# inhavl-shlee/AFI-GAN

Measured on AMD Instinct MI355X. Metric: stage1_G+D_step_images_per_s, higher is better.
Workload: dtype f32 via f16x3: two scaled fp16 pieces per operand, three f16 MFMAs per product, fp32 accumulate (tensors fp32)

## Files before the change

afigan_amd/csrc/afi_launch.h:

```cpp
#pragma once
#include "afi_common.h"

int afi_launch_pix_gemm(const AfiPixGemm& p, int b_rc, hipStream_t st);
int afi_launch_gemm_tn(const float* Q, const float* V, float* dU, int planes, long long rows_per_plane, int M, int N, hipStream_t st, bool deterministic = false);
int afi_launch_gemm_nt(const float* A, const float* B, float* C, int planes, long long rows_per_plane, int N, int K, hipStream_t st);
int afi_launch_split_bf16_tiles(const float* B, void* out, int planes, int N, int K, int split, hipStream_t st);
int afi_launch_gemm_nt_bf16_dma(const float* A, const void* Bsplit, float* C, int planes, long long rows_per_plane, int N, int K, int split, hipStream_t st);
int afi_launch_gemm_tn_bf16(const float* Q, const float* V, float* dU, int planes, long long rows_per_plane, int M, int N, int split, hipStream_t st, bool deterministic = false);
int afi_launch_split_f16_tiles(const float* B, void* out, int planes, int N, int K, hipStream_t st, int wkind = 0);
int afi_f16_image_begin(void* out, hipStream_t st);
float* afi_f16_image_wmax(void* out);
long long afi_f16_image_bytes(int planes, int N, int K);
int afi_launch_absmax_planes(const float* X, long long per_plane, int planes, float* out, hipStream_t st);
AfiF16Bound afi_f16_bound(const float* amax, int kind);
int afi_launch_gemm_nt_f16x3(const float* A, const void* Bimg, float* C, int planes, long long rows_per_plane, int N, int K, const AfiF16Bound& ab, hipStream_t st,
                             bool a_pre = false, long long nt256_min_tiles = 512, bool local_sums = false);
int afi_launch_gemm_tn_f16x3(const float* Q, const float* V, float* dU, int planes, long long rows_per_plane, int M, int N, const AfiF16Bound& qb, const AfiF16Bound& vb,
                             hipStream_t st, bool pre = false, bool deterministic = false);
int afi_launch_wgrad_gemm(const AfiWgradGemm& p, hipStream_t st);
int afi_launch_wgrad_gemm_group(const AfiWgradGemm* probs, int n, int wide, hipStream_t st);
int afi_launch_wgrad_gemm_group6(const AfiWgradGemm* probs, int n, hipStream_t st);
int afi_launch_pix_gemm_group(const AfiPixGemm* probs, int n, int b_rc, hipStream_t st);
void* afi_prof_open(hipStream_t st, int kind, double flops, long long m, int n, int k);
void afi_prof_close(void* scope);

long long afi_wk6_image_bytes(int Ncols, int Ck, int ntaps, int nKphase);
int afi_launch_wk6_images(const AfiWk6ImgJob* jobs, int n, hipStream_t st, const AfiWk6Side* side = nullptr, const AfiWk6ConvT* ct = nullptr);
int afi_launch_pix_gemm_sk(const AfiPixGemm& p, int b_rc, hipStream_t st);
int afi_launch_pix_gemm_wk_group(const AfiPixGemm* probs, int n, int b_rc, hipStream_t st);
int afi_launch_wgrad_group(const AfiWgradGemm* probs, int n, int wide, hipStream_t st);
int afi_launch_wgrad6_group(const AfiWgradGemm* probs, int n, hipStream_t st);

#define AFI_FROZEN1X1_PLAN_SLOTS 12
enum { AFI_F1_M = 0, AFI_F1_BM, AFI_F1_BN, AFI_F1_KC, AFI_F1_NTM, AFI_F1_NTN, AFI_F1_GRID, AFI_F1_LDS, AFI_F1_XBYTES, AFI_F1_OBYTES, AFI_F1_IBYTES, AFI_F1_XDENSE };

int afi_launch_nchw_to_nhwc(const float* in, float* out, int N, int C, int P, hipStream_t st);
int afi_launch_cast_to_f32_nhwc(const void* in, int dt, int N, int C, int H, int W, long long sN, long long sC, long long sH, long long sW, float* out,
                                hipStream_t st);
int afi_launch_cast_from_f32_nhwc(const AfiView& in, int N, int H, int W, int C, void* out, int dt, hipStream_t st);

int afi_launch_colsum_group(const AfiColsumProb* probs, int n, hipStream_t st);
int afi_launch_nhwc_to_nchw(const float* in, float* out, int N, int C, int P, hipStream_t st);
int afi_launch_convT_pack(const float* W, float* Wp, int Cin, int Cout, hipStream_t st);
int afi_launch_convT_unpack_grad(const float* dWp, float* dW, int Cin, int Cout, hipStream_t st);
int afi_launch_rdb_wgrad_unpack(const float* dWp, float* const dw[4], int C, int G, float alpha, hipStream_t st);
int afi_launch_rdb_wgrad_unpack_multi(const float* dWp, long long stride, float* const (*dw)[4], int nblocks, int C, int G, float alpha, hipStream_t st);
int afi_launch_g_bwd_tail(const AfiColsumProb* cs, int n_cs, const float* dWpT, float* dWT, int Cin, int Cout,
                          const float* dWp, long long stride, float* const (*dw)[4], int nblocks, int C, int G, float alpha, hipStream_t st);
int afi_launch_rdb_xpart_pack(const float* const w[4], float* out, int C, int G, hipStream_t st);
// ... 58 lines not shown
```

afigan_amd/csrc/frozen1x1.hip:

```cpp
#include "afi_common.h"
#include "afi_launch.h"
#include "afi_bf16_split.h"

#define AFI_F1_ROWS 64
struct AfiFrozen1x1 {
    const float* x; long long x_sN, x_sH, x_sW;
    const unsigned char* image; const float* bias; const float* add; float* out;
    unsigned x_bytes, o_bytes, i_bytes;
    int x_dense, M, HW, W, Cin, Cout, kc, ntile_n, nst;
    float alpha, add_scale; int act;
};

__device__ __forceinline__ int afi_f1_logical_id() {
    const int nwg = gridDim.x, qq = nwg >> 3, rr = nwg & 7, xcd = blockIdx.x & 7;
    return (xcd < rr ? xcd * (qq + 1) : rr * (qq + 1) + (xcd - rr) * qq) + (int)(blockIdx.x >> 3);
}

template <int NJ>
__global__ __launch_bounds__(256, 2) void afi_frozen1x1_kernel(const AfiFrozen1x1 p) {
    extern __shared__ __attribute__((aligned(16))) unsigned char lds[];
    const int tid = threadIdx.x, lane = tid & 63, l15 = lane & 15, lq = lane >> 4;
    const int wave = __builtin_amdgcn_readfirstlane(tid >> 6);
    const int lb = afi_f1_logical_id();
    const int tile_m = lb / p.ntile_n, tile_n = lb - tile_m * p.ntile_n;
    const int m0 = tile_m * AFI_F1_ROWS;
    const int kc = p.kc, nks = kc >> 5, nchunks = p.Cin / kc, part_bytes = kc * 128;
    const int pl = kc == 128 ? 5 : (kc == 64 ? 4 : 3);
    const int iters = 1 << (pl - 2);
    const __amdgpu_buffer_rsrc_t rsrc_x = __builtin_amdgcn_make_buffer_rsrc((void*)p.x, 0, p.x_bytes, 0x00020000);
    const __amdgpu_buffer_rsrc_t rsrc_b = __builtin_amdgcn_make_buffer_rsrc((void*)p.image, 0, p.i_bytes, 0x00020000);

    const int q = tid & ((1 << pl) - 1), r0 = tid >> pl, rstep = 256 >> pl;
    unsigned row_off[8];
// ... 79 lines not shown
                for (int mi = 0; mi < 4; ++mi) acc[j][mi] = mfma(bm, fa[mi][1], acc[j][mi]);
#pragma unroll
                for (int mi = 0; mi < 4; ++mi) acc[j][mi] = mfma(bh, fa[mi][1], acc[j][mi]);
#pragma unroll
                for (int mi = 0; mi < 4; ++mi) acc[j][mi] = mfma(bm, fa[mi][0], acc[j][mi]);
#pragma unroll
                for (int mi = 0; mi < 4; ++mi) acc[j][mi] = mfma(bh, fa[mi][0], acc[j][mi]);
            }
        }
        if (c + 1 < nchunks) __syncthreads();
    }

    const __amdgpu_buffer_rsrc_t rsrc_o = __builtin_amdgcn_make_buffer_rsrc((void*)p.out, 0, p.o_bytes, 0x00020000);
    const __amdgpu_buffer_rsrc_t rsrc_r = __builtin_amdgcn_make_buffer_rsrc((void*)p.add, 0, p.add ? p.o_bytes : 0u, 0x00020000);
    const float slope = p.act == 1 ? AFI_LRELU_SLOPE : 0.f;
#pragma unroll
    for (int j = 0; j < NJ; ++j) {
        const int col = 16 * (h0 + j) + 4 * lq;
        if (16 * (h0 + j) >= p.Cout) break;
        f32x4 bias = {0.f, 0.f, 0.f, 0.f};
        if (p.bias) bias = *(const f32x4*)(p.bias + col);
        unsigned off[4];
        f32x4 r[4];
#pragma unroll
        for (int mi = 0; mi < 4; ++mi) {
            const int m = m0 + 16 * mi + l15;
            off[mi] = m < p.M ? 4u * ((unsigned)m * (unsigned)p.Cout + (unsigned)col) : 0xFFFFFFFFu;
            r[mi] = f32x4{0.f, 0.f, 0.f, 0.f};
            if (p.add) r[mi] = __builtin_bit_cast(f32x4, __builtin_amdgcn_raw_buffer_load_b128(rsrc_r, off[mi], 0, 0));
        }
#pragma unroll
        for (int mi = 0; mi < 4; ++mi) {
            f32x4 v = p.alpha * acc[j][mi];
            v += bias;
            if (p.add) v += p.add_scale * r[mi];
            if (p.act) {
#pragma unroll
                for (int e = 0; e < 4; ++e) v[e] = v[e] > 0.f ? v[e] : v[e] * slope;
            }
            __builtin_amdgcn_raw_buffer_store_b128(__builtin_bit_cast(u32x4, v), rsrc_o, off[mi], 0, 0);
        }
    }
}

extern "C" int afi_frozen1x1_plan(int N, int H, int W, int Cin, int Cout, long long x_sN, long long x_sH, long long x_sW, long long o_sN, long long o_sH,
                                  long long o_sW, int has_add, long long a_sN, long long a_sH, long long a_sW, long long* plan) {
    if (!plan || N <= 0 || H <= 0 || W <= 0 || Cin <= 0 || Cout <= 0) return AFI_ERR_BAD_ARG;
    for (int i = 0; i < AFI_FROZEN1X1_PLAN_SLOTS; ++i) plan[i] = 0;
    if ((Cin & 31) || (Cout & 31)) return AFI_ERR_UNSUPPORTED;
    const long long kLimit = 0x7FFFFFF0LL;
    const long long M = (long long)N * H * W;
    if (M > (1LL << 30)) return AFI_ERR_UNSUPPORTED;
    if (x_sW < Cin || x_sW % Cin != 0) return AFI_ERR_UNSUPPORTED;
    const long long s = x_sW / Cin, row_span = ((long long)(W - 1) * s + 1) * Cin;
    if (H > 1 && x_sH < s * row_span) return AFI_ERR_UNSUPPORTED;
// ... 26 lines not shown

extern "C" long long afi_frozen1x1_image_bytes(int Cout, int Cin) {
    if (Cout <= 0 || Cin <= 0 || (Cout & 31) || (Cin & 31)) return 0;
    return afi_wk6_image_bytes(Cout, Cin, 1, 1);
}

extern "C" int afi_conv1x1_frozen_image(afi_ctx_t* ctx, const float* w, int Cout, int Cin, void* image, long long image_bytes, void* stream) {
    (void)ctx;
    if (!w || !image || Cout <= 0 || Cin <= 0) return AFI_ERR_BAD_ARG;
    if ((Cout & 31) || (Cin & 31)) return AFI_ERR_UNSUPPORTED;
    if (image_bytes < afi_wk6_image_bytes(Cout, Cin, 1, 1)) return AFI_ERR_WORKSPACE;
    const AfiWk6ImgJob job = {w, (long long)Cin, 0, Cout, Cin, 1, 1, 0, (unsigned char*)image};
    return afi_launch_wk6_images(&job, 1, (hipStream_t)stream);
}

extern "C" int afi_conv1x1_frozen_fwd(afi_ctx_t* ctx, afi_view_t x, int N, int H, int W, int Cin, const void* image, const float* bias, int Cout, afi_view_t out,
                                      float alpha, afi_view_t add, float add_scale, int act, void* stream) {
    (void)ctx;
    if (!x.p || !out.p || !image || act < 0 || act > 2) return AFI_ERR_BAD_ARG;
    long long plan[AFI_FROZEN1X1_PLAN_SLOTS];
    AFI_TRY(afi_frozen1x1_plan(N, H, W, Cin, Cout, x.sN, x.sH, x.sW, out.sN, out.sH, out.sW, add.p != nullptr, add.sN, add.sH, add.sW, plan));
    if ((((uintptr_t)x.p | (uintptr_t)out.p | (uintptr_t)image | (uintptr_t)add.p | (uintptr_t)bias) & 15)) return AFI_ERR_UNSUPPORTED;
    AfiFrozen1x1 p;
    p.x = x.p; p.x_sN = x.sN; p.x_sH = x.sH; p.x_sW = x.sW;
    p.image = (const unsigned char*)image; p.bias = bias; p.add = add.p; p.out = out.p;
    p.x_bytes = (unsigned)plan[AFI_F1_XBYTES]; p.o_bytes = (unsigned)plan[AFI_F1_OBYTES]; p.i_bytes = (unsigned)plan[AFI_F1_IBYTES];
    p.x_dense = (int)plan[AFI_F1_XDENSE]; p.M = (int)plan[AFI_F1_M]; p.HW = H * W; p.W = W; p.Cin = Cin; p.Cout = Cout;
    p.kc = (int)plan[AFI_F1_KC]; p.ntile_n = (int)plan[AFI_F1_NTN]; p.nst = Cin / 32;
    p.alpha = alpha; p.add_scale = add_scale; p.act = act;
    const hipStream_t st = (hipStream_t)stream;
    const dim3 grid((unsigned)plan[AFI_F1_GRID]), block(256);
    const unsigned lds = (unsigned)plan[AFI_F1_LDS];
    void* prof = afi_prof_open(st, 23, 2.0 * (double)p.M * Cin * Cout, p.M, Cout, Cin);
    switch ((int)plan[AFI_F1_BN]) {
        case 256: hipLaunchKernelGGL(afi_frozen1x1_kernel<4>, grid, block, lds, st, p); break;
        case 128: hipLaunchKernelGGL(afi_frozen1x1_kernel<2>, grid, block, lds, st, p); break;
        default:  hipLaunchKernelGGL(afi_frozen1x1_kernel<1>, grid, block, lds, st, p); break;
    }
    afi_prof_close(prof);
    return hipGetLastError() == hipSuccess ? AFI_OK : AFI_ERR_LAUNCH;
}
```

afigan_amd/csrc/nets.hip:

```cpp
#include <string.h>
#include <stdlib.h>

#include "../../include/afigan_hip.h"
#include "afi_common.h"
#include "afi_launch.h"
#include <initializer_list>
#include <new>


#include <vector>
namespace {
struct SideStream {
    hipStream_t side = nullptr;
    std::vector<hipEvent_t> ring;
    size_t next = 0;
    bool init() {
        if (side) return true;
        if (hipStreamCreateWithFlags(&side, hipStreamNonBlocking) != hipSuccess) { side = nullptr; return false; }
        ring.resize(128);
        for (auto& e : ring)
            if (hipEventCreateWithFlags(&e, hipEventDisableTiming) != hipSuccess) return false;
        return true;
    }
    void destroy() {
// ... 691 lines not shown
    if (N <= 0 || H <= 0 || W <= 0 || !ws) return AFI_ERR_BAD_ARG;
    if ((Cin & 3) || (Cout & 3)) return AFI_ERR_UNSUPPORTED;
    AfiPixGemm g = conv_fwd_desc(V(x), N, H, W, Cin, w, bias, Cout, V(out));
    g.o_dtype = out_dtype;
    return wino_run(cx, g, wino_form(cx, g, 0), ws, ws_floats, nullptr, 0, (hipStream_t)stream);
}
int afi_conv3x3_wino_infer(afi_ctx_t* ctx, afi_view_t x, int N, int H, int W, int Cin, const float* w, const float* bias, int Cout, afi_view_t out, int act,
                           float* ws, long long ws_floats, void* stream) {
    afi_ctx* cx = ctx; (void)cx;
    AFI_CTX_CHECK(ctx);
    if (N <= 0 || H <= 0 || W <= 0 || !ws || act < 0 || act > 2) return AFI_ERR_BAD_ARG;
    if ((Cin & 3) || (Cout & 3)) return AFI_ERR_UNSUPPORTED;
    AfiPixGemm g = conv_fwd_desc(V(x), N, H, W, Cin, w, bias, Cout, V(out));
    g.lrelu = act;
    return wino_run(cx, g, wino_form(cx, g, 0, true), ws, ws_floats, nullptr, 0, (hipStream_t)stream);
}
int afi_conv3x3_wino_dgrad(afi_ctx_t* ctx, afi_view_t dy, int N, int H, int W, int Cout, const float* w, int Cin, afi_view_t dx, afi_view_t z, float* ws,
                           long long ws_floats, void* stream) {
    afi_ctx* cx = ctx; (void)cx;
    AFI_CTX_CHECK(ctx);
    if (N <= 0 || H <= 0 || W <= 0 || !ws) return AFI_ERR_BAD_ARG;
    return wino_conv(cx, kWinoDgrad, V(dy), N, H, W, Cout, w, Cin, nullptr, V(dx), z.p ? V(z) : null_view(), ws, ws_floats, nullptr, 0, (hipStream_t)stream);
}

int afi_conv3x3_wino_wgrad(afi_ctx_t* ctx, afi_view_t dy, afi_view_t x, int N, int H, int W, int Cout, int Cin, float* dw, float alpha, float* ws,
                           long long ws_floats, void* stream) {
    afi_ctx* cx = ctx; (void)cx;
    AFI_CTX_CHECK(ctx);
    if (N <= 0 || H <= 0 || W <= 0 || !ws || !dw) return AFI_ERR_BAD_ARG;
    return wino_wgrad(cx, V(dy), V(x), N, H, W, Cout, Cin, dw, alpha, ws, ws_floats, (hipStream_t)stream);
// ... 1176 lines not shown
```

afigan_amd/frozen.py:

```python
import torch
import torch.nn as nn

from . import ops
from ._lib import AfiError

FROZEN_BN_EPS = 1e-5


class FrozenBatchNorm2d(nn.Module):

    def __init__(self, num_features, eps=FROZEN_BN_EPS):
        super().__init__()
        self.num_features, self.eps = num_features, eps
        self.register_buffer("weight", torch.ones(num_features))
        self.register_buffer("bias", torch.zeros(num_features))
        self.register_buffer("running_mean", torch.zeros(num_features))
        self.register_buffer("running_var", torch.ones(num_features) - eps)


def fold_conv(conv, norm=None, scale=1.0):
    w = conv.weight.detach().double()
    b = conv.bias.detach().double() if conv.bias is not None else torch.zeros(w.shape[0], dtype=torch.float64, device=w.device)
    if norm is not None:
        s = norm.weight.double() * torch.rsqrt(norm.running_var.double() + norm.eps)
# ... 25 lines not shown
def conv1x1(x, wb, stride=1, add=None, relu=False, alpha=1.0, add_scale=1.0, owner=None):
    if stride != 1:
        x = x[:, :, ::stride, ::stride]
    if add is not None and add.shape[-2:] != x.shape[-2:]:
        raise AfiError(f"resnet_guide: addend {tuple(add.shape)} does not match the conv output {tuple(x.shape[-2:])}")
    if owner is not None and ops.conv1x1_frozen_routed(x, wb[0].shape[0], add):
        return ops.conv1x1_frozen_fwd(x, conv1x1_image(owner, wb[0]), wb[1], wb[0].shape[0], add=add, add_scale=add_scale, alpha=alpha,
                                      act=2 if relu else 0)
    return ops.conv1x1_fwd(x, wb[0], wb[1], add=add, add_scale=add_scale, alpha=alpha, act=2 if relu else 0)


def conv1x1_image(module, w, name="image1x1"):
    return prepared(module, name, list(module.parameters()) + list(module.buffers()), lambda: ops.conv1x1_frozen_image(w))


def conv3x3(x, wb, stride=1, relu=False):
    act = 2 if relu else 0
    if stride == 2:
        return ops.conv3x3s2_fwd(x, wb[0], wb[1], act=act)
    N, C, H, W = x.shape
    if C >= 128 and wb[0].shape[0] >= 128 and N * H * W >= 1024:
        return ops.conv3x3_wino_infer(x, wb[0], wb[1], act=act)
    return ops.conv3x3_fwd(x, wb[0], wb[1], lrelu=act)


def prepared(module, name, tensors, build):
    key = tuple((t._version, t.data_ptr(), str(t.device)) for t in tensors)
    if getattr(module, f"_{name}_key", None) != key:
        setattr(module, f"_{name}", build())
        setattr(module, f"_{name}_key", key)
    return getattr(module, f"_{name}")


def adopt_prepared(module, name, tensors):
    if not hasattr(module, f"_{name}_key"):
        raise AfiError(f"adopt_prepared: {type(module).__name__} has no prepared slot {name!r} to adopt (prepared() builds it first)")
    setattr(module, f"_{name}_key", tuple((t._version, t.data_ptr(), str(t.device)) for t in tensors))

# ... 18 lines not shown
```

afigan_amd/guide.py:

```python
import math

import torch
import torch.nn as nn
import torch.nn.functional as F

from . import frozen, ops


def _kaiming(shape, fan_in, gain=1.0):
    return torch.randn(shape) * (gain * math.sqrt(2.0 / fan_in))


class _Conv1x1(nn.Module):
    def __init__(self, cin, cout, stride=1, relu=False, gain=1.0):
        super().__init__()
        self.stride, self.relu = stride, relu
        self.register_buffer("w", _kaiming((cin, cout), cin, gain).t().contiguous())
        self.register_buffer("b", torch.zeros(cout))

    def forward(self, x, add=None, relu=None):
        if self.stride != 1:
            x = x[:, :, ::self.stride, ::self.stride]
        act = 2 if (self.relu if relu is None else relu) else 0
        if ops.conv1x1_frozen_routed(x, self.w.shape[0], add):
            return ops.conv1x1_frozen_fwd(x, frozen.conv1x1_image(self, self.w), self.b, self.w.shape[0], add=add, act=act)
        return ops.conv1x1_fwd(x, self.w, self.b, add=add, act=act)


class _Conv3x3(nn.Module):
    def __init__(self, cin, cout, relu=False):
        super().__init__()
        self.relu = relu
        self.register_buffer("w", _kaiming((cout, 3, 3, cin), cin * 9).permute(0, 3, 1, 2))
        self.register_buffer("b", torch.zeros(cout))

    def forward(self, x):
        N, C, H, W = x.shape
        if C >= 128 and self.w.shape[0] >= 128 and N * H * W >= 1024:
            return ops.conv3x3_wino_infer(x, self.w, self.b, act=2 if self.relu else 0)
        return ops.conv3x3_fwd(x, self.w, self.b, lrelu=2 if self.relu else 0)


class _Bottleneck(nn.Module):
    def __init__(self, cin, mid, cout, stride):
        super().__init__()
        self.c1 = _Conv1x1(cin, mid, stride, relu=True)
        self.c2 = _Conv3x3(mid, mid, relu=True)
        self.c3 = _Conv1x1(mid, cout, gain=0.25)
        self.short = _Conv1x1(cin, cout, stride) if (cin != cout or stride != 1) else None

    def forward(self, x):
        s = x if self.short is None else self.short(x)
        return self.c3(self.c2(self.c1(x)), add=s, relu=True)


class GuideR50FPN(nn.Module):

    def __init__(self, out_channels=256):
        super().__init__()
        self.register_buffer("stem_w", _kaiming((3 * 49, 64), 3 * 49))
        self.register_buffer("stem_b", torch.zeros(64))
        cfg = [(64, 64, 256, 3, 1), (256, 128, 512, 4, 2), (512, 256, 1024, 6, 2), (1024, 512, 2048, 3, 2)]
        self.stages = nn.ModuleList()
        for cin, mid, cout, n, stride in cfg:
            blocks = [_Bottleneck(cin, mid, cout, stride)] + [_Bottleneck(cout, mid, cout, 1) for _ in range(n - 1)]
            self.stages.append(nn.Sequential(*blocks))
        self.lateral = nn.ModuleList([_Conv1x1(c, out_channels, gain=0.1) for c in (256, 512, 1024, 2048)])
        self.output = nn.ModuleList([_Conv3x3(out_channels, out_channels) for _ in range(4)])
        self.register_buffer("pixel_mean", torch.tensor([103.53, 116.28, 123.675]).view(1, 3, 1, 1))
        self.eval()

    @torch.no_grad()
    def forward(self, images):
        x = (images - self.pixel_mean) * (1.0 / 58.0)
        H, W = x.shape[-2:]
        ph, pw = (32 - H % 32) % 32, (32 - W % 32) % 32
        if ph or pw:
            x = F.pad(x, (0, pw, 0, ph))
        w7 = frozen.prepared(self, "stem_w7", [self.stem_w], lambda: self.stem_w.t().reshape(64, 3, 7, 7).contiguous())
        x = ops.resnet_stem(x, w7, self.stem_b)
        feats = []
        for st in self.stages:
            x = st(x)
            feats.append(x)
        prev = self.lateral[3](feats[3])
        outs = [self.output[3](prev)]
        for i in (2, 1, 0):
            up = F.interpolate(prev, scale_factor=2, mode="nearest")
            prev = self.lateral[i](feats[i], add=up)
            outs.insert(0, self.output[i](prev))
        outs.append(outs[-1][:, :, ::2, ::2].contiguous(memory_format=torch.channels_last))
        return {f"p{i + 2}": o for i, o in enumerate(outs)}
```

afigan_amd/ops.py:

```python
import contextlib
import ctypes as C
import os

import numpy as np
import torch

from . import _lib
from ._lib import View, call

_NULL_VIEW = View(None, 0, 0, 0)


def stream_ptr():
    return C.c_void_p(torch.cuda.current_stream().cuda_stream)


def _check_cuda(*ts):
    for t in ts:
        if t is None:
            continue
        if not t.is_cuda:
            raise _lib.AfiError("the AFI-GAN hot path runs on the GPU only (got a CPU tensor); there is no CPU fallback")
        if t.dtype != torch.float32:
            raise _lib.AfiError(f"fp32 only on this path, got {t.dtype}")
# ... 426 lines not shown

def conv1x1_frozen_image(w):
    global frozen1x1_images_built
    _check_cuda(w)
    Cout, Cin = w.shape[0], w.shape[1]
    w2 = w.reshape(Cout, Cin).contiguous()
    nbytes = _lib.load().afi_frozen1x1_image_bytes(Cout, Cin)
    if nbytes <= 0:
        raise _lib.AfiError(f"conv1x1_frozen_image: Cout {Cout} and Cin {Cin} must be positive multiples of 32")
    image = torch.empty(nbytes, device=w.device, dtype=torch.uint8)
    call("afi_conv1x1_frozen_image", _p(w2), Cout, Cin, _p(image), nbytes, stream_ptr())
    frozen1x1_images_built += 1
    return image


def conv1x1_frozen_fwd(x, image, bias, Cout, add=None, add_scale=1.0, alpha=1.0, out=None, act=0):
    _check_cuda(x, bias, add, out)
    N, Cin, H, W = x.shape
    if out is None:
        out = new_pixel_major(N, Cout, H, W, x.device)
    call("afi_conv1x1_frozen_fwd", view_of(x), N, H, W, Cin, _p(image), _p(bias), Cout, view_of(out), float(alpha),
         view_of(add) if add is not None else _NULL_VIEW, float(add_scale), int(act), stream_ptr())
    return out


def conv1x1_dgrad(dy, w, dx=None, alpha=1.0, beta=0.0, out_dtype=torch.float32, *, z=None, z_act="lrelu", add=None, add_scale=1.0):
    _check_cuda(dy, w, dx, z, add)
    _ensure_op_scratch(dy.device)
    N, Cout, H, W = dy.shape
    Cin = w.shape[1]
    w2 = w.reshape(Cout, Cin).contiguous()
    if z is not None or add is not None:
        if out_dtype != torch.float32:
            raise _lib.AfiError("conv1x1_dgrad: z= / add= go with an fp32 dx")
        if dx is None:
            dx = new_pixel_major(N, Cin, H, W, dy.device)
        for name, t in (("dx", dx), ("z", z), ("add", add)):
# ... 1544 lines not shown
```

afigan_amd/resnet_guide.py:

```python
import torch
import torch.nn as nn

from . import _lib, ops, registry
from ._lib import AfiError
from .fpn_sr import ShapeSpec
from .frozen import FROZEN_BN_EPS, Conv2d, FrozenBatchNorm2d, adopt_prepared, cfg_get, check_forward_only, conv1x1, conv3x3, prepared
from .rpn import _wino

_BLOCKS = {50: [3, 4, 6, 3], 101: [3, 4, 23, 3]}


class _Frozen(nn.Module):
    what = "the ResNet-FPN guide"

    def _own_convs(self):
        raise NotImplementedError

    def _fold_own(self, convs):
        return {id(m): m.fold() for m in convs}

    def _prepare_tensors(self, convs):
        return [t for m in convs for t in list(m.parameters()) + list(m.buffers())]

    def _prepare(self):
# ... 12 lines not shown

class BottleneckBlock(nn.Module):

    def __init__(self, cin, cout, bottleneck, stride, stride_in_1x1):
        super().__init__()
        self.shortcut = Conv2d(cin, cout, 1, stride=stride) if cin != cout else None
        s1, s3 = (stride, 1) if stride_in_1x1 else (1, stride)
        self.conv1 = Conv2d(cin, bottleneck, 1, stride=s1)
        self.conv2 = Conv2d(bottleneck, bottleneck, 3, stride=s3)
        self.conv3 = Conv2d(bottleneck, cout, 1)

    def run(self, x, f, route=False):
        own = (lambda m: m) if route else (lambda m: None)
        s = x if self.shortcut is None else conv1x1(x, f[id(self.shortcut)], self.shortcut.stride, owner=own(self.shortcut))
        y = conv1x1(x, f[id(self.conv1)], self.conv1.stride, relu=True, owner=own(self.conv1))
        y = conv3x3(y, f[id(self.conv2)], self.conv2.stride, relu=True)
        return conv1x1(y, f[id(self.conv3)], add=s, relu=True, owner=own(self.conv3))

    def convs(self):
        return [self.conv1, self.conv2, self.conv3] + ([self.shortcut] if self.shortcut is not None else [])

    def run_keep(self, x, f):
        s = x if self.shortcut is None else conv1x1(x, f[id(self.shortcut)], self.shortcut.stride)
        a1 = conv1x1(x, f[id(self.conv1)], self.conv1.stride, relu=True)
        a2 = conv3x3(a1, f[id(self.conv2)], self.conv2.stride, relu=True)
        return a1, a2, conv1x1(a2, f[id(self.conv3)], add=s, relu=True)


def _strided(t, stride):
    return t if stride == 1 else t[:, :, ::stride, ::stride]

# ... 314 lines not shown
    def _fold_own(self, convs):
        f = super()._fold_own(convs)
        if self._fuse_type == "avg":
            for m in self.lateral_convs[1:]:
                f[("avg", id(m))] = m.fold(scale=0.5)
        return f

    def forward(self, x):
        check_forward_only(self, x, self.what)
        feats = self.bottom_up(x)
        with torch.no_grad():
            f = self._prepare()
            xs = [feats[k] for k in self.in_features[::-1]]
            own = (lambda m: m) if getattr(self.bottom_up, "_route_frozen1x1", False) else (lambda m: None)
            prev = conv1x1(xs[0], f[id(self.lateral_convs[0])], owner=own(self.lateral_convs[0]))
            results = [conv3x3(prev, f[id(self.output_convs[0])])]
            for feat, lat, out in zip(xs[1:], self.lateral_convs[1:], self.output_convs[1:]):
                td = ops.nearest(prev, up=2)
                if self._fuse_type == "avg":
                    prev = conv1x1(feat, f[("avg", id(lat))], add=td, alpha=0.5, add_scale=0.5, owner=own(lat))
                else:
                    prev = conv1x1(feat, f[id(lat)], add=td, owner=own(lat))
                results.insert(0, conv3x3(prev, f[id(out)]))
            results.append(ops.nearest(results[-1], up=1, down=2))
        return dict(zip(self._out_features, results))


def _resnet_from_cfg(cfg, input_shape=None):
    r = cfg_get(cfg.MODEL, "RESNETS", None)
    if input_shape is not None and getattr(input_shape, "channels", 3) not in (None, 3):
        raise AfiError(f"resnet_guide: 3 input channels only, got {input_shape.channels}")
    norm = cfg_get(r, "NORM", "FrozenBN")
    if norm != "FrozenBN":
        raise AfiError(f"resnet_guide: RESNETS.NORM {norm!r} is not supported (the frozen guide folds FrozenBN)")
    if cfg_get(r, "NUM_GROUPS", 1) != 1:
        raise AfiError(f"resnet_guide: RESNETS.NUM_GROUPS {cfg_get(r, 'NUM_GROUPS', 1)} is not supported (groups = 1 only)")
    if cfg_get(r, "RES5_DILATION", 1) != 1:
        raise AfiError(f"resnet_guide: RESNETS.RES5_DILATION {cfg_get(r, 'RES5_DILATION', 1)} is not supported (no dilation)")
# ... 31 lines not shown
```

include/afigan_hip.h:

```cpp
#ifndef AFIGAN_HIP_H
#define AFIGAN_HIP_H

#include <stddef.h>
#include <stdint.h>

#ifdef __cplusplus
extern "C" {
#endif

#define AFI_OK 0
#define AFI_ERR_BAD_ARG 1
#define AFI_ERR_UNSUPPORTED 2
#define AFI_ERR_LAUNCH 3
#define AFI_ERR_WORKSPACE 4

#define AFI_MAX_RDB 8

typedef struct afi_view {
    float* p;
    long long sN, sH, sW;
} afi_view_t;

int afi_abi_version(void);
const char* afi_status_string(int status);
// ... 212 lines not shown
long long afi_dual_scale_u8_ws_bytes(int H0, int W0, int C, int H1, int W1, int H2, int W2);
int afi_dual_scale_u8(const unsigned char* src, int H0, int W0, int C, unsigned char* image, int H1, int W1, int hflip,
                      unsigned char* image_r, int H2, int W2, int hflip_r, int out_chw, void* ws, long long ws_bytes, void* stream);
int afi_normalize_pad_u8(const unsigned char* img_chw, int C, int H, int W, const float* mean, const float* std_,
                         float* out, int Hp, int Wp, void* stream);

int afi_resnet_stem_fwd(const float* x, int N, int H, int W, const float* w, const float* bias, float* out, void* stream);
int afi_nearest_nhwc(afi_view_t x, int N, int H, int W, int C, int up, int down, float* out, void* stream);

long long afi_frozen1x1_image_bytes(int Cout, int Cin);
int afi_frozen1x1_plan(int N, int H, int W, int Cin, int Cout, long long x_sN, long long x_sH, long long x_sW, long long o_sN, long long o_sH,
                       long long o_sW, int has_add, long long a_sN, long long a_sH, long long a_sW, long long* plan);
int afi_conv1x1_frozen_image(afi_ctx_t* ctx, const float* w, int Cout, int Cin, void* image, long long image_bytes, void* stream);
int afi_conv1x1_frozen_fwd(afi_ctx_t* ctx, afi_view_t x, int N, int H, int W, int Cin, const void* image, const float* bias, int Cout, afi_view_t out,
                           float alpha, afi_view_t add_or_null, float add_scale, int act, void* stream);

#define AFI_POOL_MAX3S2P1 0
#define AFI_POOL_AVG3S2P1 1
#define AFI_POOL_AVG2S2_CEIL 2
int afi_resnest_stem_fwd(const float* x, int N, int H, int W, const float* w, const float* bias, int Cout, float* out, void* stream);
int afi_resnest_pool_nhwc(afi_view_t x, int N, int H, int W, int C, int mode, float* out, void* stream);
long long afi_resnest_splat_ws_floats(int N, int H, int W, int C);
int afi_resnest_splat_gap(afi_view_t s0, afi_view_t s1, int N, int H, int W, int C, float* part, long long part_floats, void* stream);
int afi_resnest_splat_attn(const float* part, int N, int H, int W, int C, int I, const float* w1, const float* b1, const float* w2,
                           const float* b2, float* att, void* stream);
int afi_resnest_splat_combine(afi_view_t s0, afi_view_t s1, int N, int H, int W, int C, const float* att, int avd, float* out, void* stream);

int afi_resnest_splat_attn_keep(const float* part, int N, int H, int W, int C, int I, const float* w1, const float* b1, const float* w2,
                                const float* b2, float* att, float* g, float* h, void* stream);
long long afi_resnest_splat_bwd_ws_floats(int N, int H, int W, int C);
// ... 163 lines not shown
```

Before: 29.53.

## Cache Winograd fp16 weight images for frozen 3x3 convs and fuse input absmax

Adds a frozen 3x3 Winograd path for the guide network. It builds the split-fp16 weight image once per module and caches it, so the weight transform and split no longer run on every forward. The preceding frozen 1x1 conv can now emit the absmax of its output through an atomic max in its epilogue. The 3x3 conv then reuses that value instead of running a separate absmax reduction over its input. The cost is a new workspace allocation per call, a small extra reduction in the 1x1 epilogue, and a cache of images that becomes stale if the weights change.

```diff
diff --git a/afigan_amd/csrc/afi_launch.h b/afigan_amd/csrc/afi_launch.h
--- a/afigan_amd/csrc/afi_launch.h
+++ b/afigan_amd/csrc/afi_launch.h
@@ -33,6 +33,9 @@
 
 #define AFI_FROZEN1X1_PLAN_SLOTS 12
 enum { AFI_F1_M = 0, AFI_F1_BM, AFI_F1_BN, AFI_F1_KC, AFI_F1_NTM, AFI_F1_NTN, AFI_F1_GRID, AFI_F1_LDS, AFI_F1_XBYTES, AFI_F1_OBYTES, AFI_F1_IBYTES, AFI_F1_XDENSE };
+
+#define AFI_FROZEN3X3_PLAN_SLOTS 8
+enum { AFI_F3_F4 = 0, AFI_F3_PLANES, AFI_F3_T, AFI_F3_TPAD, AFI_F3_IBYTES, AFI_F3_WSFLOATS, AFI_F3_TILE, AFI_F3_PRESPLIT };
 
 int afi_launch_nchw_to_nhwc(const float* in, float* out, int N, int C, int P, hipStream_t st);
 int afi_launch_cast_to_f32_nhwc(const void* in, int dt, int N, int C, int H, int W, long long sN, long long sC, long long sH, long long sW, float* out,
diff --git a/afigan_amd/csrc/frozen1x1.hip b/afigan_amd/csrc/frozen1x1.hip
--- a/afigan_amd/csrc/frozen1x1.hip
+++ b/afigan_amd/csrc/frozen1x1.hip
@@ -9,6 +9,7 @@
     unsigned x_bytes, o_bytes, i_bytes;
     int x_dense, M, HW, W, Cin, Cout, kc, ntile_n, nst;
     float alpha, add_scale; int act;
+    float* out_amax;
 };
 
 __device__ __forceinline__ int afi_f1_logical_id() {
@@ -16,7 +17,7 @@
     return (xcd < rr ? xcd * (qq + 1) : rr * (qq + 1) + (xcd - rr) * qq) + (int)(blockIdx.x >> 3);
 }
 
-template <int NJ>
+template <int NJ, bool AMAX = false>
 __global__ __launch_bounds__(256, 2) void afi_frozen1x1_kernel(const AfiFrozen1x1 p) {
     extern __shared__ __attribute__((aligned(16))) unsigned char lds[];
     const int tid = threadIdx.x, lane = tid & 63, l15 = lane & 15, lq = lane >> 4;
@@ -126,6 +127,7 @@
     const __amdgpu_buffer_rsrc_t rsrc_o = __builtin_amdgcn_make_buffer_rsrc((void*)p.out, 0, p.o_bytes, 0x00020000);
     const __amdgpu_buffer_rsrc_t rsrc_r = __builtin_amdgcn_make_buffer_rsrc((void*)p.add, 0, p.add ? p.o_bytes : 0u, 0x00020000);
     const float slope = p.act == 1 ? AFI_LRELU_SLOPE : 0.f;
+    float vmax = 0.f;
 #pragma unroll
     for (int j = 0; j < NJ; ++j) {
         const int col = 16 * (h0 + j) + 4 * lq;
@@ -151,6 +153,18 @@
                 for (int e = 0; e < 4; ++e) v[e] = v[e] > 0.f ? v[e] : v[e] * slope;
             }
             __builtin_amdgcn_raw_buffer_store_b128(__builtin_bit_cast(u32x4, v), rsrc_o, off[mi], 0, 0);
+            if (AMAX && off[mi] != 0xFFFFFFFFu) vmax = fmaxf(fmaxf(vmax, fmaxf(fabsf(v[0]), fabsf(v[1]))), fmaxf(fabsf(v[2]), fabsf(v[3])));
+        }
+    }
+    if constexpr (AMAX) {
+        __shared__ float red[4];
+#pragma unroll
+        for (int o = 32; o > 0; o >>= 1) vmax = fmaxf(vmax, __shfl_xor(vmax, o));
+        if (lane == 0) red[wave] = vmax;
+        __syncthreads();
+        if (tid == 0) {
+            const unsigned bits = __float_as_uint(fmaxf(fmaxf(red[0], red[1]), fmaxf(red[2], red[3])));
+            if (bits > __hip_atomic_load((const unsigned*)p.out_amax, __ATOMIC_RELAXED, __HIP_MEMORY_SCOPE_AGENT)) (void)atomicMax((unsigned*)p.out_amax, bits);
         }
     }
 }
@@ -207,9 +221,8 @@
     return afi_launch_wk6_images(&job, 1, (hipStream_t)stream);
 }
 
-extern "C" int afi_conv1x1_frozen_fwd(afi_ctx_t* ctx, afi_view_t x, int N, int H, int W, int Cin, const void* image, const float* bias, int Cout, afi_view_t out,
-                                      float alpha, afi_view_t add, float add_scale, int act, void* stream) {
-    (void)ctx;
+static int frozen1x1_fwd(afi_view_t x, int N, int H, int W, int Cin, const void* image, const float* bias, int Cout, afi_view_t out, float alpha, afi_view_t add,
+                        float add_scale, int act, float* out_amax, void* stream) {
     if (!x.p || !out.p || !image || act < 0 || act > 2) return AFI_ERR_BAD_ARG;
     long long plan[AFI_FROZEN1X1_PLAN_SLOTS];
     AFI_TRY(afi_frozen1x1_plan(N, H, W, Cin, Cout, x.sN, x.sH, x.sW, out.sN, out.sH, out.sW, add.p != nullptr, add.sN, add.sH, add.sW, plan));
@@ -220,16 +233,32 @@
     p.x_bytes = (unsigned)plan[AFI_F1_XBYTES]; p.o_bytes = (unsigned)plan[AFI_F1_OBYTES]; p.i_bytes = (unsigned)plan[AFI_F1_IBYTES];
     p.x_dense = (int)plan[AFI_F1_XDENSE]; p.M = (int)plan[AFI_F1_M]; p.HW = H * W; p.W = W; p.Cin = Cin; p.Cout = Cout;
     p.kc = (int)plan[AFI_F1_KC]; p.ntile_n = (int)plan[AFI_F1_NTN]; p.nst = Cin / 32;
-    p.alpha = alpha; p.add_scale = add_scale; p.act = act;
+    p.alpha = alpha; p.add_scale = add_scale; p.act = act; p.out_amax = out_amax;
     const hipStream_t st = (hipStream_t)stream;
     const dim3 grid((unsigned)plan[AFI_F1_GRID]), block(256);
     const unsigned lds = (unsigned)plan[AFI_F1_LDS];
     void* prof = afi_prof_open(st, 23, 2.0 * (double)p.M * Cin * Cout, p.M, Cout, Cin);
-    switch ((int)plan[AFI_F1_BN]) {
-        case 256: hipLaunchKernelGGL(afi_frozen1x1_kernel<4>, grid, block, lds, st, p); break;
-        case 128: hipLaunchKernelGGL(afi_frozen1x1_kernel<2>, grid, block, lds, st, p); break;
-        default:  hipLaunchKernelGGL(afi_frozen1x1_kernel<1>, grid, block, lds, st, p); break;
+    const int bn = (int)plan[AFI_F1_BN];
+    if (out_amax) {
+        if (bn == 256) hipLaunchKernelGGL((afi_frozen1x1_kernel<4, true>), grid, block, lds, st, p);
+        else if (bn == 128) hipLaunchKernelGGL((afi_frozen1x1_kernel<2, true>), grid, block, lds, st, p);
+        else hipLaunchKernelGGL((afi_frozen1x1_kernel<1, true>), grid, block, lds, st, p);
+    } else {
+        if (bn == 256) hipLaunchKernelGGL(afi_frozen1x1_kernel<4>, grid, block, lds, st, p);
+        else if (bn == 128) hipLaunchKernelGGL(afi_frozen1x1_kernel<2>, grid, block, lds, st, p);
+        else hipLaunchKernelGGL(afi_frozen1x1_kernel<1>, grid, block, lds, st, p);
     }
     afi_prof_close(prof);
     return hipGetLastError() == hipSuccess ? AFI_OK : AFI_ERR_LAUNCH;
 }
+extern "C" int afi_conv1x1_frozen_fwd(afi_ctx_t* ctx, afi_view_t x, int N, int H, int W, int Cin, const void* image, const float* bias, int Cout, afi_view_t out,
+                                      float alpha, afi_view_t add, float add_scale, int act, void* stream) {
+    (void)ctx;
+    return frozen1x1_fwd(x, N, H, W, Cin, image, bias, Cout, out, alpha, add, add_scale, act, nullptr, stream);
+}
+extern "C" int afi_conv1x1_frozen_fwd_amax(afi_ctx_t* ctx, afi_view_t x, int N, int H, int W, int Cin, const void* image, const float* bias, int Cout,
+                                           afi_view_t out, float alpha, afi_view_t add, float add_scale, int act, float* out_amax, void* stream) {
+    (void)ctx;
+    if (!out_amax || ((uintptr_t)out_amax & 3)) return AFI_ERR_BAD_ARG;
+    return frozen1x1_fwd(x, N, H, W, Cin, image, bias, Cout, out, alpha, add, add_scale, act, out_amax, stream);
+}
diff --git a/afigan_amd/csrc/nets.hip b/afigan_amd/csrc/nets.hip
--- a/afigan_amd/csrc/nets.hip
+++ b/afigan_amd/csrc/nets.hip
@@ -729,6 +729,69 @@
     AfiPixGemm g = conv_fwd_desc(V(x), N, H, W, Cin, w, bias, Cout, V(out));
     g.lrelu = act;
     return wino_run(cx, g, wino_form(cx, g, 0, true), ws, ws_floats, nullptr, 0, (hipStream_t)stream);
+}
+
+constexpr long long kFrozen3x3SlotFloats = 64;
+static int frozen3x3_plan(const afi_ctx* cx, int N, int H, int W, int Cin, int Cout, long long* plan, WinoForm* form = nullptr) {
+    if (!plan || N <= 0 || H <= 0 || W <= 0 || Cin <= 0 || Cout <= 0) return AFI_ERR_BAD_ARG;
+    for (int i = 0; i < AFI_FROZEN3X3_PLAN_SLOTS; ++i) plan[i] = 0;
+    const long long P = (long long)N * H * W, kLimit = 0x7FFFFFF0LL;
+    if (Cin < 128 || Cout < 128 || P > (1LL << 30)) return AFI_ERR_UNSUPPORTED;
+    const WinoForm f = wino_form(cx, N, H, W, Cin, Cout, kWinoFwdF4);
+    if (!(f.dma && f.f16)) return AFI_ERR_UNSUPPORTED;
+    const long long v = align4(f.np * f.Tpad * Cin), m = align4(f.np * f.Tpad * Cout), img = afi_f16_image_bytes(f.np, Cout, Cin);
+    if (4 * v >= kLimit || 4 * m >= kLimit || img >= kLimit || 4 * P * Cin >= kLimit || 4 * P * Cout >= kLimit) return AFI_ERR_UNSUPPORTED;
+    const long long nt256 = afi_opt(cx, AFI_OPT_F16_NT256_MIN_TILES);
+    const bool t256 = nt256 > 0 && !(Cout % 256) && (long long)f.np * afi_cdiv(f.Tpad, 256) * (Cout / 256) >= nt256;
+    plan[AFI_F3_F4] = f.f4 ? 1 : 0; plan[AFI_F3_PLANES] = f.np; plan[AFI_F3_T] = f.T; plan[AFI_F3_TPAD] = f.Tpad;
+    plan[AFI_F3_IBYTES] = img; plan[AFI_F3_WSFLOATS] = v + m + kFrozen3x3SlotFloats; plan[AFI_F3_TILE] = t256 ? 256 : 128;
+    plan[AFI_F3_PRESPLIT] = f.presplit ? 1 : 0;
+    if (form) *form = f;
+    return P >= 1024 || form ? AFI_OK : AFI_ERR_UNSUPPORTED;
+}
+int afi_frozen3x3_plan(const afi_ctx_t* ctx, int N, int H, int W, int Cin, int Cout, long long* plan) { return frozen3x3_plan(ctx, N, H, W, Cin, Cout, plan); }
+int afi_frozen3x3_plan_dtype(int dtype, int N, int H, int W, int Cin, int Cout, long long* plan) {
+    if (!afi_dtype_ok(dtype)) return AFI_ERR_BAD_ARG;
+    afi_ctx cx;
+    cx.dtype = dtype;
+    return frozen3x3_plan(&cx, N, H, W, Cin, Cout, plan);
+}
+int afi_conv3x3_frozen_image(afi_ctx_t* ctx, const float* w, int Cin, int Cout, int f4, void* image, long long image_bytes, void* stream) {
+    (void)ctx;
+    if (!w || !image || Cin <= 0 || Cout <= 0 || (f4 != 0 && f4 != 1)) return AFI_ERR_BAD_ARG;
+    if ((Cout % 128) || (Cin % 32)) return AFI_ERR_UNSUPPORTED;
+    if (image_bytes < afi_f16_image_bytes(f4 ? 36 : 16, Cout, Cin)) return AFI_ERR_WORKSPACE;
+    const AfiWinoImgJob job{w, (unsigned char*)image, Cout, Cin, f4, 0};
+    return afi_launch_wino_weight_images(&job, 1, afi_f16_image_wmax(image), (hipStream_t)stream);
+}
+int afi_conv3x3_frozen_fwd(afi_ctx_t* ctx, afi_view_t x, int N, int H, int W, int Cin, const void* image, int f4, const float* bias, int Cout, afi_view_t out,
+                           int act, float* in_amax, float* ws, long long ws_floats, void* stream) {
+    afi_ctx* cx = ctx;
+    AFI_CTX_CHECK(ctx);
+    if (!x.p || !out.p || !image || !ws || act < 0 || act > 2) return AFI_ERR_BAD_ARG;
+    long long plan[AFI_FROZEN3X3_PLAN_SLOTS];
+    WinoForm f;
+    AFI_TRY(frozen3x3_plan(cx, N, H, W, Cin, Cout, plan, &f));
+    if (f4 != (int)plan[AFI_F3_F4]) return AFI_ERR_BAD_ARG;
+    if (ws_floats < plan[AFI_F3_WSFLOATS]) return AFI_ERR_WORKSPACE;
+    if ((((uintptr_t)image | (uintptr_t)ws) & 15) || ((uintptr_t)in_amax & 3)) return AFI_ERR_UNSUPPORTED;
+    const hipStream_t st = (hipStream_t)stream;
+    AfiPixGemm g = conv_fwd_desc(V(x), N, H, W, Cin, nullptr, bias, Cout, V(out));
+    g.lrelu = act;
+    const int np = f.np; const long long Tpad = f.Tpad;
+    float* Vb = ws;
+    float* Mb = Vb + align4(np * Tpad * Cin);
+    float* amax = in_amax;
+    if (!amax) {
+        amax = Mb + align4(np * Tpad * Cout);
+        if (hipMemsetAsync(amax, 0, sizeof(float) * kFrozen3x3SlotFloats, st) != hipSuccess) return AFI_ERR_LAUNCH;
+    }
+    const bool a_pre = in_amax && f.presplit;
+    const AfiF16Bound abound = afi_f16_bound(amax, f.f4 ? 2 : 1);
+    AFI_TRY(f.f4 ? afi_launch_wino4_input(g.A, N, H, W, Cin, Tpad, Vb, st, Cin, in_amax ? nullptr : amax, a_pre ? &abound : nullptr)
+                 : afi_launch_wino_input(g.A, N, H, W, Cin, Tpad, Vb, st, Cin, in_amax ? nullptr : amax, a_pre ? &abound : nullptr));
+    AFI_TRY(afi_launch_gemm_nt_f16x3(Vb, image, Mb, np, Tpad, Cout, Cin, abound, st, a_pre, afi_opt(cx, AFI_OPT_F16_NT256_MIN_TILES), false));
+    return f.f4 ? afi_launch_wino4_output_epi(Mb, Tpad, g, st) : afi_launch_wino_output_epi(Mb, Tpad, g, st);
 }
 int afi_conv3x3_wino_dgrad(afi_ctx_t* ctx, afi_view_t dy, int N, int H, int W, int Cout, const float* w, int Cin, afi_view_t dx, afi_view_t z, float* ws,
                            long long ws_floats, void* stream) {
diff --git a/afigan_amd/frozen.py b/afigan_amd/frozen.py
--- a/afigan_amd/frozen.py
+++ b/afigan_amd/frozen.py
@@ -63,14 +63,22 @@
     return prepared(module, name, list(module.parameters()) + list(module.buffers()), lambda: ops.conv1x1_frozen_image(w))
 
 
-def conv3x3(x, wb, stride=1, relu=False):
+def conv3x3(x, wb, stride=1, relu=False, owner=None, in_amax=None):
     act = 2 if relu else 0
     if stride == 2:
         return ops.conv3x3s2_fwd(x, wb[0], wb[1], act=act)
     N, C, H, W = x.shape
     if C >= 128 and wb[0].shape[0] >= 128 and N * H * W >= 1024:
+        plan = ops.conv3x3_frozen_routed(x, wb[0].shape[0]) if owner is not None else None
+        if plan is not None:
+            return ops.conv3x3_frozen_fwd(x, conv3x3_image(owner, wb[0], plan["f4"]), plan["f4"], wb[1], wb[0].shape[0], act=act, in_amax=in_amax)
         return ops.conv3x3_wino_infer(x, wb[0], wb[1], act=act)
     return ops.conv3x3_fwd(x, wb[0], wb[1], lrelu=act)
+
+
+def conv3x3_image(module, w, f4):
+    return prepared(module, "image3x3_f4" if f4 else "image3x3_f2", list(module.parameters()) + list(module.buffers()),
+                    lambda: ops.conv3x3_frozen_image(w, f4))
 
 
 def prepared(module, name, tensors, build):
diff --git a/afigan_amd/guide.py b/afigan_amd/guide.py
--- a/afigan_amd/guide.py
+++ b/afigan_amd/guide.py
@@ -18,13 +18,15 @@
         self.register_buffer("w", _kaiming((cin, cout), cin, gain).t().contiguous())
         self.register_buffer("b", torch.zeros(cout))
 
-    def forward(self, x, add=None, relu=None):
+    def forward(self, x, add=None, relu=None, amax=None):
         if self.stride != 1:
             x = x[:, :, ::self.stride, ::self.stride]
         act = 2 if (self.relu if relu is None else relu) else 0
         if ops.conv1x1_frozen_routed(x, self.w.shape[0], add):
-            return ops.conv1x1_frozen_fwd(x, frozen.conv1x1_image(self, self.w), self.b, self.w.shape[0], add=add, act=act)
-        return ops.conv1x1_fwd(x, self.w, self.b, add=add, act=act)
+            out = ops.conv1x1_frozen_fwd(x, frozen.conv1x1_image(self, self.w), self.b, self.w.shape[0], add=add, act=act, out_amax=amax)
+            return out if amax is None else (out, amax)
+        out = ops.conv1x1_fwd(x, self.w, self.b, add=add, act=act)
+        return out if amax is None else (out, None)
 
 
 class _Conv3x3(nn.Module):
@@ -34,11 +36,15 @@
         self.register_buffer("w", _kaiming((cout, 3, 3, cin), cin * 9).permute(0, 3, 1, 2))
         self.register_buffer("b", torch.zeros(cout))
 
-    def forward(self, x):
+    def forward(self, x, in_amax=None):
         N, C, H, W = x.shape
+        act = 2 if self.relu else 0
         if C >= 128 and self.w.shape[0] >= 128 and N * H * W >= 1024:
-            return ops.conv3x3_wino_infer(x, self.w, self.b, act=2 if self.relu else 0)
-        return ops.conv3x3_fwd(x, self.w, self.b, lrelu=2 if self.relu else 0)
+            plan = ops.conv3x3_frozen_routed(x, self.w.shape[0])
+            if plan is not None:
+                return ops.conv3x3_frozen_fwd(x, frozen.conv3x3_image(self, self.w, plan["f4"]), plan["f4"], self.b, self.w.shape[0], act=act, in_amax=in_amax)
+            return ops.conv3x3_wino_infer(x, self.w, self.b, act=act)
+        return ops.conv3x3_fwd(x, self.w, self.b, lrelu=act)
 
 
 class _Bottleneck(nn.Module):
@@ -49,9 +55,10 @@
         self.c3 = _Conv1x1(mid, cout, gain=0.25)
         self.short = _Conv1x1(cin, cout, stride) if (cin != cout or stride != 1) else None
 
-    def forward(self, x):
+    def forward(self, x, amax=None):
         s = x if self.short is None else self.short(x)
-        return self.c3(self.c2(self.c1(x)), add=s, relu=True)
+        a1, known = self.c1(x, amax=amax) if amax is not None else (self.c1(x), None)
+        return self.c3(self.c2(a1, in_amax=known), add=s, relu=True)
 
 
 class GuideR50FPN(nn.Module):
@@ -79,15 +86,18 @@
             x = F.pad(x, (0, pw, 0, ph))
         w7 = frozen.prepared(self, "stem_w7", [self.stem_w], lambda: self.stem_w.t().reshape(64, 3, 7, 7).contiguous())
         x = ops.resnet_stem(x, w7, self.stem_b)
-        feats = []
+        slots = ops.amax_slots(20, x.device)
+        feats, k = [], 0
         for st in self.stages:
-            x = st(x)
+            for blk in st:
+                x = blk(x, amax=ops.amax_slot(slots, k))
+                k += 1
             feats.append(x)
-        prev = self.lateral[3](feats[3])
-        outs = [self.output[3](prev)]
+        prev, known = self.lateral[3](feats[3], amax=ops.amax_slot(slots, 19))
+        outs = [self.output[3](prev, in_amax=known)]
         for i in (2, 1, 0):
             up = F.interpolate(prev, scale_factor=2, mode="nearest")
-            prev = self.lateral[i](feats[i], add=up)
-            outs.insert(0, self.output[i](prev))
+            prev, known = self.lateral[i](feats[i], add=up, amax=ops.amax_slot(slots, 16 + i))
+            outs.insert(0, self.output[i](prev, in_amax=known))
         outs.append(outs[-1][:, :, ::2, ::2].contiguous(memory_format=torch.channels_last))
         return {f"p{i + 2}": o for i, o in enumerate(outs)}
diff --git a/afigan_amd/ops.py b/afigan_amd/ops.py
--- a/afigan_amd/ops.py
+++ b/afigan_amd/ops.py
@@ -464,13 +464,80 @@
     return image
 
 
-def conv1x1_frozen_fwd(x, image, bias, Cout, add=None, add_scale=1.0, alpha=1.0, out=None, act=0):
-    _check_cuda(x, bias, add, out)
+def conv1x1_frozen_fwd(x, image, bias, Cout, add=None, add_scale=1.0, alpha=1.0, out=None, act=0, out_amax=None):
+    _check_cuda(x, bias, add, out, out_amax)
     N, Cin, H, W = x.shape
     if out is None:
         out = new_pixel_major(N, Cout, H, W, x.device)
-    call("afi_conv1x1_frozen_fwd", view_of(x), N, H, W, Cin, _p(image), _p(bias), Cout, view_of(out), float(alpha),
-         view_of(add) if add is not None else _NULL_VIEW, float(add_scale), int(act), stream_ptr())
+    add_v = view_of(add) if add is not None else _NULL_VIEW
+    if out_amax is not None:
+        call("afi_conv1x1_frozen_fwd_amax", view_of(x), N, H, W, Cin, _p(image), _p(bias), Cout, view_of(out), float(alpha), add_v, float(add_scale),
+             int(act), _p(out_amax), stream_ptr())
+        return out
+    call("afi_conv1x1_frozen_fwd", view_of(x), N, H, W, Cin, _p(image), _p(bias), Cout, view_of(out), float(alpha), add_v, float(add_scale), int(act),
+         stream_ptr())
+    return out
+
+
+frozen3x3_route = True
+frozen3x3_images_built = 0
+AMAX_SLOT_STRIDE = 4
+_F3_PLAN = ("f4", "planes", "T", "Tpad", "image_bytes", "ws_floats", "tile", "presplit")
+
+
+def amax_slots(n, device):
+    return torch.zeros((n * AMAX_SLOT_STRIDE + 63) // 64 * 64, device=device, dtype=torch.float32)
+
+
+def amax_slot(buf, i):
+    return buf[i * AMAX_SLOT_STRIDE:i * AMAX_SLOT_STRIDE + 1]
+
+
+def conv3x3_frozen_plan(N, H, W, Cin, Cout, dtype=None, small_maps=False):
+    plan = (C.c_longlong * len(_F3_PLAN))()
+    if dtype is None:
+        st = _lib.load().afi_frozen3x3_plan(_lib.current_ctx().handle, N, H, W, Cin, Cout, plan)
+    else:
+        st = _lib.load().afi_frozen3x3_plan_dtype(_lib.DTYPES[dtype], N, H, W, Cin, Cout, plan)
+    if st == _lib.DEFINES["AFI_ERR_UNSUPPORTED"]:
+        return dict(zip(_F3_PLAN, plan)) if small_maps and plan[1] else None
+    _lib.check(st, "afi_frozen3x3_plan")
+    return dict(zip(_F3_PLAN, plan))
+
+
+def conv3x3_frozen_routed(x, Cout):
+    if not frozen3x3_route or not x.is_cuda or x.dtype != torch.float32 or not is_pixel_major(x):
+        return None
+    N, Cin, H, W = x.shape
+    return conv3x3_frozen_plan(N, H, W, Cin, Cout)
+
+
+def conv3x3_frozen_image(w, f4):
+    global frozen3x3_images_built
+    _check_cuda(w)
+    Cout, Cin = w.shape[0], w.shape[1]
+    if Cout % 128 or Cin % 32:
+        raise _lib.AfiError(f"conv3x3_frozen_image: Cout {Cout} must be a multiple of 128 and Cin {Cin} of 32")
+    w = ohwi(w)
+    nbytes = 512 + (36 if f4 else 16) * Cin * Cout * 4
+    image = torch.empty(nbytes, device=w.device, dtype=torch.uint8)
+    call("afi_conv3x3_frozen_image", _p(w), Cin, Cout, int(bool(f4)), _p(image), nbytes, stream_ptr())
+    frozen3x3_images_built += 1
+    return image
+
+
+def conv3x3_frozen_fwd(x, image, f4, bias, Cout, act=0, in_amax=None, out=None):
+    _check_cuda(x, bias, in_amax, out)
+    N, Cin, H, W = x.shape
+    plan = conv3x3_frozen_plan(N, H, W, Cin, Cout, small_maps=True)
+    if plan is None:
+        raise _lib.AfiError(f"conv3x3_frozen_fwd: the plan refuses {tuple(x.shape)} -> {Cout} channels under {_lib.current_ctx().dtype} "
+                            "(callers ask conv3x3_frozen_routed first and take conv3x3_wino_infer otherwise)")
+    ws = new_workspace(plan["ws_floats"], x.device)
+    if out is None:
+        out = new_pixel_major(N, Cout, H, W, x.device)
+    call("afi_conv3x3_frozen_fwd", view_of(x), N, H, W, Cin, _p(image), int(bool(f4)), _p(bias), Cout, view_of(out), int(act), _p(in_amax), _p(ws),
+         plan["ws_floats"], stream_ptr())
     return out
 
 
diff --git a/afigan_amd/resnet_guide.py b/afigan_amd/resnet_guide.py
--- a/afigan_amd/resnet_guide.py
+++ b/afigan_amd/resnet_guide.py
@@ -50,7 +50,7 @@
         own = (lambda m: m) if route else (lambda m: None)
         s = x if self.shortcut is None else conv1x1(x, f[id(self.shortcut)], self.shortcut.stride, owner=own(self.shortcut))
         y = conv1x1(x, f[id(self.conv1)], self.conv1.stride, relu=True, owner=own(self.conv1))
-        y = conv3x3(y, f[id(self.conv2)], self.conv2.stride, relu=True)
+        y = conv3x3(y, f[id(self.conv2)], self.conv2.stride, relu=True, owner=own(self.conv2))
         return conv1x1(y, f[id(self.conv3)], add=s, relu=True, owner=own(self.conv3))
 
     def convs(self):
@@ -395,14 +395,14 @@
             xs = [feats[k] for k in self.in_features[::-1]]
             own = (lambda m: m) if getattr(self.bottom_up, "_route_frozen1x1", False) else (lambda m: None)
             prev = conv1x1(xs[0], f[id(self.lateral_convs[0])], owner=own(self.lateral_convs[0]))
-            results = [conv3x3(prev, f[id(self.output_convs[0])])]
+            results = [conv3x3(prev, f[id(self.output_convs[0])], owner=own(self.output_convs[0]))]
             for feat, lat, out in zip(xs[1:], self.lateral_convs[1:], self.output_convs[1:]):
                 td = ops.nearest(prev, up=2)
                 if self._fuse_type == "avg":
                     prev = conv1x1(feat, f[("avg", id(lat))], add=td, alpha=0.5, add_scale=0.5, owner=own(lat))
                 else:
                     prev = conv1x1(feat, f[id(lat)], add=td, owner=own(lat))
-                results.insert(0, conv3x3(prev, f[id(out)]))
+                results.insert(0, conv3x3(prev, f[id(out)], owner=own(out)))
             results.append(ops.nearest(results[-1], up=1, down=2))
         return dict(zip(self._out_features, results))
 
diff --git a/include/afigan_hip.h b/include/afigan_hip.h
--- a/include/afigan_hip.h
+++ b/include/afigan_hip.h
@@ -250,6 +250,14 @@
 int afi_conv1x1_frozen_image(afi_ctx_t* ctx, const float* w, int Cout, int Cin, void* image, long long image_bytes, void* stream);
 int afi_conv1x1_frozen_fwd(afi_ctx_t* ctx, afi_view_t x, int N, int H, int W, int Cin, const void* image, const float* bias, int Cout, afi_view_t out,
                            float alpha, afi_view_t add_or_null, float add_scale, int act, void* stream);
+int afi_conv1x1_frozen_fwd_amax(afi_ctx_t* ctx, afi_view_t x, int N, int H, int W, int Cin, const void* image, const float* bias, int Cout, afi_view_t out,
+                                float alpha, afi_view_t add_or_null, float add_scale, int act, float* out_amax, void* stream);
+
+int afi_frozen3x3_plan(const afi_ctx_t* ctx, int N, int H, int W, int Cin, int Cout, long long* plan);
+int afi_frozen3x3_plan_dtype(int dtype, int N, int H, int W, int Cin, int Cout, long long* plan);
+int afi_conv3x3_frozen_image(afi_ctx_t* ctx, const float* w_ohwi, int Cin, int Cout, int f4, void* image, long long image_bytes, void* stream);
+int afi_conv3x3_frozen_fwd(afi_ctx_t* ctx, afi_view_t x, int N, int H, int W, int Cin, const void* image, int f4, const float* bias_or_null, int Cout,
+                           afi_view_t out, int act, float* in_amax_or_null, float* ws, long long ws_floats, void* stream);
 
 #define AFI_POOL_MAX3S2P1 0
 #define AFI_POOL_AVG3S2P1 1
```

Result: no change. 29.61 (median of 6 runs) (+0.3%).
